# carry4985/ORB_SLAM2_MAP

Hardware: AMD Instinct MI355X
Metric: frames/sec ORB extract+match (640x480, 1000 feat) (higher is better)
Workload: dtype u8; 1 GPU; C2: synthetic 640x480 RGB-D stream, 1000 features, 8 levels, extract + BF-Hamming match of consecutive frames; resident_frame_pool=1024, sequences=1, parallelism=1 sequence per GPU, schedule_name=best, extraction_parts=1

## Files before the change

### include/orbgpu.h

```cpp
#ifndef ORBGPU_H
#define ORBGPU_H

#include <stddef.h>
#include <stdint.h>

#ifdef __cplusplus
extern "C" {
#endif

#define ORBGPU_ABI_VERSION 1
#define ORBGPU_MAX_LEVELS 16

typedef enum {
    ORBGPU_OK = 0,
    ORBGPU_EINVAL = -1,
    ORBGPU_ENOMEM = -2,
    ORBGPU_EHIP = -3,
    ORBGPU_ECAPACITY = -4,
    ORBGPU_ELEVEL = -5
} orbgpu_status;

const char *orbgpu_last_error_string(void);
int orbgpu_abi_version(void);
int orbgpu_device_count(void);
// ... 43 lines not shown
                         size_t stride, size_t frame_stride, orbgpu_keypoint *kps, uint8_t *desc, int32_t cap,
                         int32_t *n_out);

int orbgpu_extract_batch_device(orbgpu_extractor *h, const uint8_t *d_gray, int32_t batch, int32_t width,
                                int32_t height, size_t stride, size_t frame_stride, orbgpu_keypoint *d_kps,
                                uint8_t *d_desc, int32_t cap, int32_t *d_n_out, void *hip_stream);

int orbgpu_extractor_get_pyramid_level(orbgpu_extractor *h, int32_t frame, int32_t level, uint8_t *dst,
                                       size_t dst_stride, int32_t *width, int32_t *height);

enum {
    ORBGPU_DBG_PYRAMID_PADDED = 0,
    ORBGPU_DBG_BLURRED_PADDED = 1,
    ORBGPU_DBG_CANDIDATES = 2,
    ORBGPU_DBG_SELECTED = 3,
    ORBGPU_DBG_GRAPH_COUNTS = 4
};
int orbgpu_extractor_debug_read(orbgpu_extractor *h, int32_t what, int32_t frame, int32_t level, void *dst,
                                size_t dst_bytes, size_t *n, int32_t *aux);

int orbgpu_extractor_graph_state(const orbgpu_extractor *h, int32_t *state);
int orbgpu_extractor_debug_quadtree_config(const orbgpu_extractor *h, int32_t batch, int32_t *lds_keys, int32_t *threads,
                                           int32_t *lds_bytes);
int orbgpu_extractor_set_profiling(orbgpu_extractor *h, int32_t enable);
int orbgpu_extractor_set_concurrent_blur(orbgpu_extractor *h, int32_t enable);
int orbgpu_extractor_set_fast_early_out(orbgpu_extractor *h, int32_t enable);

int orbgpu_extractor_set_stage_signal(orbgpu_extractor *h, int32_t stage, void *hip_event);
int orbgpu_extractor_stage_count(void);
const char *orbgpu_extractor_stage_name(int32_t i);
int orbgpu_extractor_stage_times(orbgpu_extractor *h, float *ms_out);
// ... 388 lines not shown
```

### orb_slam2_map_amd/csrc/extractor.hip

```cpp
#include "common.h"

#include <atomic>
#include <chrono>
#include <thread>
#include <tuple>
#include <type_traits>
#include <utility>
#include "trig_base.h"
#include "pyramid_view.h"

#include <algorithm>
#include <cfloat>
#include <cmath>
#include <cstdlib>
#include <cstring>
#include <vector>

namespace orbgpu {

constexpr int EDGE = 19;
constexpr int BORDER0 = EDGE - 3;
constexpr int HALF_PATCH = 15;
constexpr int PATCH = 31;
constexpr float CELL_W = 30.f;
// ... 865 lines not shown
    __syncthreads();
    }
    __syncthreads();
    for (int i = tid; i < 4 * n_ini; i += 256)
        if (s_cnt[i])
            atomicAdd(&laux[1 + i], s_cnt[i]);
}

template <bool LDS_KEYS>
__global__ __launch_bounds__(QT_THREADS) void k_quadtree(const LevelGeom *__restrict__ geom,
                                                  const CellDesc *__restrict__ cells, int ncells_total,
                                                  const uint32_t *__restrict__ slots, size_t frame_slots,
                                                  int *__restrict__ cell_cnt,
                                                  uint32_t *__restrict__ dense_key,
                                                  uint16_t *__restrict__ dense_node,
                                                  uint32_t *__restrict__ sel, int sel_cap_total,
                                                  int *__restrict__ nsel, int *__restrict__ ncand, int nlevels,
                                                  int ncap, int t_ini, int kcap_arg, long long *dbg_t,
                                                  int *__restrict__ pre_aux )
{
#ifdef ORBGPU_QT_TIMING
    int dbg_k = 0;
#define QT_MARK(id) if (dbg_t && threadIdx.x == 0 && blockIdx.y == 0 && blockIdx.x == 0 && dbg_k < 500) { dbg_t[2 * dbg_k] = (id); dbg_t[2 * dbg_k + 1] = (long long)wall_clock64(); dbg_k++; }
#else
#define QT_MARK(id)
#endif

    extern __shared__ __align__(16) uint8_t smem[];
    __shared__ int s_tmp[16];
    const int kcap = LDS_KEYS ? kcap_arg : 0;
    __shared__ int s_n, s_phase, s_done, s_nexp, s_cut, s_nst, s_nk;
// ... 426 lines not shown
                nd[u] = node_of(i, key[u]);
            }
#pragma unroll
            for (int u = 0; u < QT_ILP; u++)
                if (i0 + u * nt < nkeys)
                    atomicMax(&best[nd[u]], best_of(key[u]));
        }
    }
    __syncthreads();
    uint32_t *osel = sel + (size_t)f * sel_cap_total + g.sel_off;
    const bool ok = done_cur != 2 && n <= g.sel_cap;
    for (int p = tid; p < n && ok; p += nt) {
        const unsigned long long b = best[p];
        const uint32_t yx = (uint32_t)((0xFFFFFFFFFFull - (b & 0xFFFFFFFFFFull)) & 0xFFFFFFull);
        osel[p] = (yx << 8) | (uint32_t)((b >> 40) - 1ull);
    }
    QT_MARK(4)
    if (tid == 0)
        nsel[(size_t)f * nlevels + level] = ok ? n : -1;
}

struct KpAux {
    int x, y, level;
    float angle;
    float ca, sb;
    int plane_off, pitch;
};

__device__ __forceinline__ float fast_atan2_deg(float y, float x)
{
// ... 15 lines not shown
        a = 180.f - a;
    if (y < 0)
        a = 360.f - a;
    return a;
}

struct UMax {
    int v[16];
};

constexpr int OR_ITERS = 4;
constexpr int OR_BATCH_MIN = 32;

__global__ __launch_bounds__(256) void k_orient(const uint8_t *__restrict__ pyr, size_t frame_pyr,
                                                const LevelGeom *__restrict__ geom, int nlevels,
                                                const uint32_t *__restrict__ sel, int sel_cap_total,
                                                const int *__restrict__ nsel, const uint32_t *__restrict__ orw,
                                                orbgpu_keypoint *__restrict__ kps, KpAux *__restrict__ aux,
                                                int cap, int *__restrict__ n_out, int iters, Src0 s0)
{
    __shared__ uint32_t W10[4 * 16 * 9], M01[4 * 16 * 9];
    __shared__ __align__(16) uint8_t stage[8][31 * 48];
    for (int i = threadIdx.x; i < 4 * 16 * 9; i += 256) {
        W10[i] = orw[i];
        M01[i] = orw[4 * 16 * 9 + i];
    }
    __syncthreads();

    const int hl = threadIdx.x & 31;
    int bx, f;
    xcd_frame_block(bx, f);
    f = serpentine(f);
    const int *ns = nsel + (size_t)f * nlevels;
    for (int it = 0; it < iters; it++) {
    const int slot = (bx * iters + it) * 8 + (threadIdx.x >> 5);
    int level = -1, j = 0, out_off = 0, total = 0, cnt_l = 0;
    bool bad = false;
// ... 11 lines not shown
            j = slot - so;
            out_off = total;
            cnt_l = c;
            g.plane_off = geom[l].plane_off;
            g.pitch = geom[l].pitch;
            g.sel_off = so;
            g.patch = geom[l].patch;
            g.scale = geom[l].scale;
        }
        total += max(c, 0);
    }
    if (slot == 0 && hl == 0)
        n_out[f] = bad ? -1 - total : (total > cap ? -1 - total : total);
    if (level < 0 || bad || total > cap || j >= cnt_l)
        continue;
    const uint32_t key = sel[(size_t)f * sel_cap_total + g.sel_off + j];
    const int x = key_x(key) + BORDER0, y = key_y(key) + BORDER0;
    const bool dir0 = s0.direct != 0 && level == 0;
    const int porg = dir0 ? 0 : EDGE, ppitch = dir0 ? (int)s0.pitch : g.pitch;
    const int xl = x + porg - HALF_PATCH;
    const int a = xl & 3;
    const int v = hl - HALF_PATCH;
    int m10 = 0, m01 = 0;
    {
        const uint8_t *base = (dir0 ? s0.p + (size_t)f * s0.frame_stride : pyr + (size_t)f * frame_pyr + g.plane_off) + (xl - a);
        struct __attribute__((packed, aligned(4))) Piece {
            uint32_t d[4];
        };
        const int lim = a == 2 ? 3 : (a == 3 ? 6 : -1);
        const uint8_t *rowbase = base + rowoff(y + porg - HALF_PATCH, ppitch);
        uint4 *pl = reinterpret_cast<uint4 *>(stage[threadIdx.x >> 5]);
// ... 42 lines not shown
    }
    if (hl == 0) {
        const float angle = fast_atan2_deg((float)m01, (float)m10);
        orbgpu_keypoint kp;
        kp.x = (float)x;
        kp.y = (float)y;
        if (level != 0) {
            kp.x *= g.scale;
            kp.y *= g.scale;
        }
        kp.size = (float)g.patch;
        kp.angle = angle;
        kp.response = (float)key_resp(key);
        kp.octave = level;
        kp.class_id = -1;
        kps[(size_t)f * cap + out_off + j] = kp;
        KpAux ax;
        ax.x = x + (dir0 ? BLUR0_OX - EDGE : 0);
        ax.y = y;
        ax.level = level;
        ax.plane_off = g.plane_off;
        ax.pitch = g.pitch;
        ax.angle = angle;
        aux[(size_t)f * cap + out_off + j] = ax;
    }
    }
}
__global__ __launch_bounds__(256) void k_trig(KpAux *__restrict__ aux, const int *__restrict__ n_out, int cap, TrigTable tt)
{
    const int f = blockIdx.y;
    const int i = blockIdx.x * 256 + threadIdx.x;
    if (i >= n_out[f])
        return;
    KpAux *a = aux + (size_t)f * cap + i;
    const float factorPI = (float)(3.14159265358979323846 / 180.f);
    const float angle = a->angle * factorPI;
    float c, s;
    orbgpu_trig_device(angle, tt, &c, &s);
    a->ca = c;
    a->sb = s;
}

constexpr int BLUR_ROWS = 30;

__device__ __forceinline__ void blur_hsum(uint32_t d0, uint32_t d1, uint32_t d2, uint32_t h[4])
{
#define W4(a, b, c, d) ((uint32_t)(a) | ((uint32_t)(b) << 8) | ((uint32_t)(c) << 16) | ((uint32_t)(d) << 24))
    h[0] = __builtin_amdgcn_udot4(d1, W4(55, 49, 34, 18), __builtin_amdgcn_udot4(d0, W4(0, 18, 34, 49), 0u, false), false);
    h[1] = __builtin_amdgcn_udot4(d2, W4(18, 0, 0, 0), __builtin_amdgcn_udot4(d1, W4(49, 55, 49, 34), __builtin_amdgcn_udot4(d0, W4(0, 0, 18, 34), 0u, false), false), false);
    h[2] = __builtin_amdgcn_udot4(d2, W4(34, 18, 0, 0), __builtin_amdgcn_udot4(d1, W4(34, 49, 55, 49), __builtin_amdgcn_udot4(d0, W4(0, 0, 0, 18), 0u, false), false), false);
    h[3] = __builtin_amdgcn_udot4(d2, W4(49, 34, 18, 0), __builtin_amdgcn_udot4(d1, W4(18, 34, 49, 55), 0u, false), false);
#undef W4
}

__device__ __forceinline__ uint32_t blur_vsum(const uint32_t A[4], const uint32_t C[4], const uint32_t E[4],
// ... 172 lines not shown
        B8_STEP(p5, p1, p3, p4, k + 5)
    }
#undef B8_PAIR
#undef B8_STEP
#undef B8_LOAD
#undef B8_HSUM
}

constexpr int DP_R = 18;
constexpr int DP_ROWS = 2 * DP_R + 1;
constexpr int DP_DW = 12;
constexpr int DP_BYTES = DP_ROWS * DP_DW * 4;

__global__ __launch_bounds__(256) void k_describe(const uint8_t *__restrict__ blur, size_t frame_pyr,
                                                  const LevelGeom *__restrict__ geom,
                                                  const KpAux *__restrict__ aux, const int *__restrict__ n_out,
                                                  int cap, const int8_t *__restrict__ pattern,
                                                  uint8_t *__restrict__ desc)
{
    __shared__ __align__(16) uint8_t patch[8][DP_BYTES];
    int bx, f;
    xcd_frame_block(bx, f);
    const int n = n_out[f];
    const int slot = threadIdx.x >> 5;
    const int kpi = bx * 8 + slot;
    if (kpi >= n)
        return;
    const int byte = threadIdx.x & 31;
    const KpAux a = aux[(size_t)f * cap + kpi];
    const uint4 pq0 = reinterpret_cast<const uint4 *>(pattern)[byte * 2];
    const uint4 pq1 = reinterpret_cast<const uint4 *>(pattern)[byte * 2 + 1];
    const uint32_t pw[8] = {pq0.x, pq0.y, pq0.z, pq0.w, pq1.x, pq1.y, pq1.z, pq1.w};
    const float ca = a.ca, sb = a.sb;
    const int xl = a.x + EDGE - DP_R;
    const int al = xl & 3;
    const uint8_t *fb = blur + (size_t)f * frame_pyr;
    const uint32_t vbase = (uint32_t)a.plane_off + (uint32_t)(a.y + EDGE - DP_R) * (uint32_t)a.pitch + (uint32_t)(xl - al);
    struct __attribute__((packed, aligned(4))) Piece {
        uint32_t d[4];
    };
    constexpr int NPIECE = DP_ROWS * 3, NK = (NPIECE + 31) / 32;
    Piece stage[NK];
#pragma unroll
    for (int k = 0; k < NK; k++) {
// ... 12 lines not shown
    constexpr float MAGIC = 12582912.0f;
    constexpr uint32_t BIAS = 0x400000u * (DP_DW * 4) + 0x4B400000u;
    const uint32_t kc = (uint32_t)(slot * DP_BYTES + DP_R * (DP_DW * 4) + DP_R + al) - BIAS;
    const uint8_t *lds = &patch[0][0];
    int val = 0;
#pragma unroll
    for (int k = 0; k < 8; k++) {
        const float x0 = (float)(int8_t)(pw[k] & 0xFF), y0 = (float)(int8_t)((pw[k] >> 8) & 0xFF);
        const float x1 = (float)(int8_t)((pw[k] >> 16) & 0xFF), y1 = (float)(int8_t)(pw[k] >> 24);
        const uint32_t r0b = __float_as_uint((x0 * sb + y0 * ca) + MAGIC), c0b = __float_as_uint((x0 * ca - y0 * sb) + MAGIC);
        const uint32_t r1b = __float_as_uint((x1 * sb + y1 * ca) + MAGIC), c1b = __float_as_uint((x1 * ca - y1 * sb) + MAGIC);
        const int t0 = lds[__umul24(r0b, DP_DW * 4) + c0b + kc];
        const int t1 = lds[__umul24(r1b, DP_DW * 4) + c1b + kc];
        val |= (t0 < t1) << k;
    }
    desc[((size_t)f * cap + kpi) * 32 + byte] = (uint8_t)val;
}

__global__ void k_unpack_keys(const uint32_t *__restrict__ keys, int n, int *__restrict__ out)
{
    int i = blockIdx.x * blockDim.x + threadIdx.x;
    if (i < n) {
        uint32_t k = keys[i];
        out[3 * i] = key_x(k);
        out[3 * i + 1] = key_y(k);
        out[3 * i + 2] = key_resp(k);
    }
}

static const int8_t k_pattern_host[1024] = {
#include "orbgpu_pattern.inc"
// ... 35 lines not shown
    int nlevels;
    float scale[ORBGPU_MAX_LEVELS], inv_scale[ORBGPU_MAX_LEVELS], sigma2[ORBGPU_MAX_LEVELS],
        inv_sigma2[ORBGPU_MAX_LEVELS];
    int quota[ORBGPU_MAX_LEVELS];
    UMax umax;
    int cfg_w = 0, cfg_h = 0, cfg_batch = 0;
    std::vector<LevelGeom> geom;
    std::vector<CellDesc> cells;
    StripGeom blur_geom;
    DetectGeom det_geom;
    size_t frame_pyr = 0, frame_slots = 0;
    int sel_cap_total = 0, ncap = 0, max_kp = 0;
    size_t qt_lds = 0;
    int qt_kcap = 0;
    DevBuf d_geom, d_cells, d_xtab, d_ytab, d_yrow, d_pattern, d_rstrip, d_rsel, d_rwt, d_ctab, d_bcol;
    DevBuf d_pyr, d_blur, d_slots, d_cellcnt, d_dkey, d_dnode, d_sel, d_nsel, d_ncand, d_aux;
    mutable DevBuf d_stereo;
    DevBuf d_qtaux;
    bool qt_prefilter = false;
    int max_slots_level = 0;
    DevBuf d_in, d_kps, d_desc, d_nout;
    void *h_pin = nullptr;
    size_t h_pin_bytes = 0;
    bool pinned_staging = true;
    DevBuf d_dbg;
    hipStream_t stream = nullptr;
    int last_batch = 0, last_cap = 0;
    static constexpr int PROF_SLOTS = 256;
    bool profiling = false;
    std::vector<hipEvent_t> ev;
    int prof_calls = 0;
// ... 7 lines not shown
    hipEvent_t stage_signal[8] = {nullptr, nullptr, nullptr, nullptr, nullptr, nullptr, nullptr, nullptr};
    hipEvent_t pipe_signal[8] = {};
    bool counters_dirty = false;
    bool force_batch_quadtree = false;
    bool concurrent_blur = false;
    hipStream_t side = nullptr;
    hipEvent_t ev_fork = nullptr, ev_fork0 = nullptr, ev_join = nullptr;
    bool qt_no_prefilter = false;
    int qt_keys_hook = -1;
    int fast_queue_cap = FD_QCAP;
    bool fast_early_out = false;
    int graph_state = 0;
    bool direct0_ok = false;
    bool no_early_blur0 = false;
    int direct0_min_batch = 8;
    bool no_direct0 = false;
    int rs_off_direct = 0;
    DetectGeom det_geom_direct;
    Src0 last_src = {nullptr, 0, 0u, 0};
    bool level0_materialized = true;
    TrigTable trig = {nullptr, nullptr, nullptr, 0u};

};

namespace orbgpu {

int trig_table_for_device(int device_id, TrigTable *out);

static void build_tables(orbgpu_extractor *e)
{
// ... 424 lines not shown
    RSV(e->d_xtab, sizeof(XTab) * std::max<size_t>(xtab.size(), 1));
    RSV(e->d_ytab, sizeof(YTab) * std::max<size_t>(ytab.size(), 1));
    RSV(e->d_yrow, sizeof(YRow) * std::max<size_t>(yrow.size(), 1));
    RSV(e->d_rstrip, sizeof(ResizeStrip) * std::max<size_t>(rstrip.size(), 1));
    RSV(e->d_rsel, sizeof(uint4) * std::max<size_t>(rsel.size(), 1));
    RSV(e->d_rwt, sizeof(uint4) * std::max<size_t>(rwt.size(), 1));
    RSV(e->d_pattern, 1024 + 2 * 4 * 16 * 9 * sizeof(uint32_t));
    const size_t B = (size_t)batch;
    RSV(e->d_pyr, e->frame_pyr * B);
    RSV(e->d_blur, e->frame_pyr * B);
    RSV(e->d_slots, sizeof(uint32_t) * e->frame_slots * B);
    RSV(e->d_cellcnt, sizeof(int) * (cells.size() + ORBGPU_MAX_LEVELS) * B);
    RSV(e->d_dkey, sizeof(uint32_t) * e->frame_slots * B);
    RSV(e->d_dnode, sizeof(uint16_t) * e->frame_slots * B);
    RSV(e->d_sel, sizeof(uint32_t) * (size_t)sel_off * B);
    RSV(e->d_nsel, sizeof(int) * nl * B);
    RSV(e->d_ncand, sizeof(int) * nl * B);
    RSV(e->d_qtaux, sizeof(int) * QT_AUX_FRAME * QT_BATCH_MIN);
#undef RSV
    ORBGPU_HIP_TRY(hipMemcpyAsync(e->d_geom.p, geom.data(), sizeof(LevelGeom) * nl, hipMemcpyHostToDevice, e->stream));
    ORBGPU_HIP_TRY(hipMemcpyAsync(e->d_cells.p, cells.data(), sizeof(CellDesc) * cells.size(), hipMemcpyHostToDevice, e->stream));
    ORBGPU_HIP_TRY(hipMemcpyAsync(e->d_ctab.p, ctab.data(), sizeof(ColumnInfo) * ctab.size(), hipMemcpyHostToDevice, e->stream));
    if (!bcol.empty())
        ORBGPU_HIP_TRY(hipMemcpyAsync(e->d_bcol.p, bcol.data(), sizeof(BorderCol) * bcol.size(), hipMemcpyHostToDevice, e->stream));
    e->border_fast = !bcol.empty();
    if (!xtab.empty()) {
        ORBGPU_HIP_TRY(hipMemcpyAsync(e->d_xtab.p, xtab.data(), sizeof(XTab) * xtab.size(), hipMemcpyHostToDevice, e->stream));
        ORBGPU_HIP_TRY(hipMemcpyAsync(e->d_ytab.p, ytab.data(), sizeof(YTab) * ytab.size(), hipMemcpyHostToDevice, e->stream));
        ORBGPU_HIP_TRY(hipMemcpyAsync(e->d_yrow.p, yrow.data(), sizeof(YRow) * yrow.size(), hipMemcpyHostToDevice, e->stream));
        ORBGPU_HIP_TRY(hipMemcpyAsync(e->d_rstrip.p, rstrip.data(), sizeof(ResizeStrip) * rstrip.size(), hipMemcpyHostToDevice, e->stream));
// ... 128 lines not shown
    if (e->blur_geom.first[nl] > strip0)
        L.launch(k_blur, dim3((e->blur_geom.first[nl] - strip0 + 255) / 256, batch), dim3(256), 0, pyr, blur,
                           e->frame_pyr, dg, e->blur_geom, strip0);
}

static int launch_pipeline(orbgpu_extractor *e, const uint8_t *d_gray, int batch, int w, int h, size_t stride,
                           size_t frame_stride, orbgpu_keypoint *d_kps, uint8_t *d_desc, int cap, int *d_n_out,
                           Launcher &L)
{
    hipStream_t st = L.st;
    const int nl = e->nlevels;
    const LevelGeom *dg = e->d_geom.as<LevelGeom>();
    uint8_t *pyr = e->d_pyr.as<uint8_t>();
    uint8_t *blur = e->d_blur.as<uint8_t>();
    int rc = e->d_aux.reserve(sizeof(KpAux) * (size_t)cap * batch);
    if (rc != ORBGPU_OK)
        return rc;
    const bool rec = L.graph != nullptr;
    const bool prof = !rec && e->profiling && e->prof_calls < orbgpu_extractor::PROF_SLOTS;
    if (prof && e->ev.empty()) {
        e->ev.resize((size_t)orbgpu_extractor::PROF_SLOTS * 2 * ST_COUNT, nullptr);
        for (auto &x : e->ev)
            ORBGPU_HIP_TRY(hipEventCreate(&x));
    }
    hipEvent_t *evs = prof ? &e->ev[(size_t)e->prof_calls * 2 * ST_COUNT] : nullptr;
#define BEGIN(stage, s) if (prof && (stage) == 0) ORBGPU_HIP_TRY(hipEventRecord(evs[0], s))
#define END(stage, s)                                                          \
    {                                                                          \
        if (prof)                                                              \
            ORBGPU_HIP_TRY(hipEventRecord(evs[1 + (stage)], s));               \
// ... 69 lines not shown
    {
        const int t_ini = std::max(e->prm.ini_th_fast, 1), t_min = std::max(e->prm.min_th_fast, 1);
        const DetectGeom &dgeo = direct ? e->det_geom_direct : e->det_geom;
        const int nwaves = (dgeo.first[nl] + FD_OWN - 1) / FD_OWN;
        L.launch(e->fast_early_out ? k_fast_detect<true> : k_fast_detect<false>, dim3((nwaves + 3) / 4, batch), dim3(256), 0, pyr, e->frame_pyr, dg,
                           dgeo, e->d_ctab.as<ColumnInfo>(), e->d_cells.as<CellDesc>(), (int)e->cells.size(),
                           e->d_slots.as<uint32_t>(), e->frame_slots, e->d_cellcnt.as<int>(), std::min(t_ini, t_min),
                           t_ini, e->fast_queue_cap, s0);
    }
    END(ST_FAST, st);
    BEGIN(ST_QUADTREE, st);
    if (batch >= QT_BATCH_MIN || e->force_batch_quadtree)
        L.launch(k_quadtree<false>, dim3(batch, nl), dim3(QT_THREADS_BATCH), e->qt_lds, dg,
                           e->d_cells.as<CellDesc>(), (int)e->cells.size(), e->d_slots.as<uint32_t>(), e->frame_slots,
                           e->d_cellcnt.as<int>(), e->d_dkey.as<uint32_t>(), e->d_dnode.as<uint16_t>(),
                           e->d_sel.as<uint32_t>(), e->sel_cap_total, e->d_nsel.as<int>(), e->d_ncand.as<int>(), nl,
                           e->ncap, std::max(e->prm.ini_th_fast, 1), 0, qt_dbg(), (int *)nullptr);
    else {
        if (e->qt_prefilter)
            L.launch(k_qt_prefilter, dim3(std::min((e->max_slots_level + QT_PRE_KEYS - 1) / QT_PRE_KEYS, QT_PRE_GRID), nl, batch), dim3(256), 0, dg, (int)e->cells.size(), e->d_slots.as<uint32_t>(), e->frame_slots, e->d_cellcnt.as<int>(),
                               e->d_dkey.as<uint32_t>(), e->d_qtaux.as<int>(), std::max(e->prm.ini_th_fast, 1));
        L.launch(k_quadtree<true>, dim3(batch, nl), dim3(w * h >= QT_LARGE_PIXELS ? QT_THREADS : QT_THREADS_SMALL), e->qt_lds + (size_t)e->qt_kcap * 6, dg,
                           e->d_cells.as<CellDesc>(), (int)e->cells.size(), e->d_slots.as<uint32_t>(), e->frame_slots,
                           e->d_cellcnt.as<int>(), e->d_dkey.as<uint32_t>(), e->d_dnode.as<uint16_t>(),
                           e->d_sel.as<uint32_t>(), e->sel_cap_total, e->d_nsel.as<int>(), e->d_ncand.as<int>(), nl,
                           e->ncap, std::max(e->prm.ini_th_fast, 1), e->qt_kcap, qt_dbg(),
                           e->qt_prefilter ? e->d_qtaux.as<int>() : (int *)nullptr);
    }
    if (!rec)
        ORBGPU_HIP_TRY(hipGetLastError());
    e->counters_dirty = false;
    END(ST_QUADTREE, st);
    BEGIN(ST_ORIENT, st);
    const int or_iters = batch >= OR_BATCH_MIN ? OR_ITERS : 1;
    L.launch(k_orient, dim3((e->sel_cap_total + 8 * or_iters - 1) / (8 * or_iters), batch), dim3(256), 0, pyr, e->frame_pyr, dg, nl,
                       e->d_sel.as<uint32_t>(), e->sel_cap_total, e->d_nsel.as<int>(),
                       reinterpret_cast<const uint32_t *>(e->d_pattern.as<uint8_t>() + 1024), d_kps,
                       e->d_aux.as<KpAux>(), cap, d_n_out, or_iters, s0);
    L.launch(k_trig, dim3((std::min(cap, e->max_kp) + 255) / 256, batch), dim3(256), 0,
                       e->d_aux.as<KpAux>(), d_n_out, cap, e->trig);
    END(ST_ORIENT, st);
    BEGIN(ST_DESCRIBE, st);
    if (side_blur)
        ORBGPU_HIP_TRY(hipStreamWaitEvent(st, e->ev_join, 0));
    L.launch(k_describe, dim3((std::min(cap, e->max_kp) + 7) / 8, batch), dim3(256), 0, blur,
                       e->frame_pyr, dg, e->d_aux.as<KpAux>(), d_n_out, cap, e->d_pattern.as<int8_t>(), d_desc);
    END(ST_DESCRIBE, st);
#undef BEGIN
#undef END
    if (!rec)
        ORBGPU_HIP_TRY(hipGetLastError());
    else if (L.err != hipSuccess) {
        set_error("recording the extraction graph: %s", hipGetErrorString(L.err));
        return ORBGPU_EHIP;
    }
    if (prof)
        e->prof_calls++;
    e->last_batch = batch;
    e->last_cap = cap;
    (void)w;
    (void)h;
// ... 51 lines not shown
    if (rc != ORBGPU_OK)
        return rc;
    orbgpu_extractor *e = new (std::nothrow) orbgpu_extractor();
    if (!e) {
        set_error("out of host memory");
        return ORBGPU_ENOMEM;
    }
    e->prm = *p;
    if (e->prm.max_batch < 1)
        e->prm.max_batch = 1;
    e->force_batch_quadtree = getenv("ORBGPU_DEBUG_QT_BATCH") != nullptr;
    e->qt_no_prefilter = getenv("ORBGPU_DEBUG_QT_NOPRE") != nullptr;
    if (const char *q = getenv("ORBGPU_DEBUG_QT_KEYS"))
        e->qt_keys_hook = std::max(atoi(q), 0);
    e->no_direct0 = getenv("ORBGPU_DEBUG_NO_DIRECT0") != nullptr;
    e->no_early_blur0 = getenv("ORBGPU_DEBUG_NO_EARLY_BLUR0") != nullptr;
    if (const char *q = getenv("ORBGPU_DEBUG_DIRECT0_MIN"))
        e->direct0_min_batch = std::max(atoi(q), 1);
    if (const char *q = getenv("ORBGPU_FAST_EARLY_OUT"))
        e->fast_early_out = atoi(q) != 0;
    e->pinned_staging = getenv("ORBGPU_DEBUG_NO_PINNED") == nullptr;
    if (getenv("ORBGPU_DEBUG_NO_GRAPH"))
        e->graph_state = -1;
    if (const char *q = getenv("ORBGPU_DEBUG_FAST_QUEUE"))
        e->fast_queue_cap = std::min(std::max(atoi(q), 0), FD_QCAP);
    e->nlevels = p->nlevels;
    build_tables(e);
    hipError_t he = hipStreamCreateWithFlags(&e->stream, hipStreamNonBlocking);
    if (he != hipSuccess) {
        set_error("hipStreamCreate: %s", hipGetErrorString(he));
// ... 7 lines not shown
        return rc;
    }
    *out = e;
    return ORBGPU_OK;
}

int orbgpu_extractor_destroy(orbgpu_extractor *e)
{
    std::lock_guard<std::mutex> lifecycle(orbgpu::lifecycle_mutex());
    if (!e)
        return ORBGPU_OK;
    (void)hipSetDevice(e->prm.device_id);
    (void)hipDeviceSynchronize();
    DevBuf *bufs[] = {&e->d_geom, &e->d_cells, &e->d_xtab, &e->d_ytab, &e->d_yrow, &e->d_pattern, &e->d_rstrip, &e->d_rsel,
                      &e->d_rwt, &e->d_ctab, &e->d_bcol, &e->d_pyr,
                      &e->d_blur, &e->d_slots, &e->d_cellcnt, &e->d_dkey, &e->d_dnode, &e->d_sel, &e->d_nsel,
                      &e->d_ncand, &e->d_aux, &e->d_in, &e->d_kps, &e->d_desc, &e->d_nout, &e->d_dbg, &e->d_qtaux, &e->d_stereo};
    for (DevBuf *b : bufs)
        b->release();
    for (auto &x : e->ev)
        if (x)
            (void)hipEventDestroy(x);
    if (e->graph_exec)
        (void)hipGraphExecDestroy(e->graph_exec);
    if (e->graph)
        (void)hipGraphDestroy(e->graph);
    if (e->h_pin)
        (void)hipHostFree(e->h_pin);
    if (e->stream)
        (void)hipStreamDestroy(e->stream);
    if (e->side)
        (void)hipStreamDestroy(e->side);
// ... 87 lines not shown
    const size_t img = (size_t)w * h;
    if (img * batch > e->d_in.bytes)
        forget_last_call(e);
    if ((rc = e->d_in.reserve(img * batch)) != ORBGPU_OK)
        return rc;
    if ((rc = e->d_kps.reserve(sizeof(orbgpu_keypoint) * (size_t)cap * batch)) != ORBGPU_OK)
        return rc;
    if ((rc = e->d_desc.reserve((size_t)32 * cap * batch)) != ORBGPU_OK)
        return rc;
    if ((rc = e->d_nout.reserve(sizeof(int) * batch)) != ORBGPU_OK)
        return rc;
    if ((rc = configure(e, w, h, std::max(batch, e->prm.max_batch))) != ORBGPU_OK)
        return rc;
    if ((rc = e->d_aux.reserve(sizeof(KpAux) * (size_t)cap * batch)) != ORBGPU_OK)
        return rc;
    uint8_t *pin_in = nullptr;
    int *pin_n = nullptr;
    orbgpu_keypoint *pin_k = nullptr;
    uint8_t *pin_d = nullptr;
    const size_t pin_need = ((img * batch + 255) & ~(size_t)255) + ((sizeof(int) * batch + 255) & ~(size_t)255) +
                            (sizeof(orbgpu_keypoint) + 32) * (size_t)cap * batch;
    if (e->pinned_staging && pin_need <= ((size_t)64 << 20)) {
        const size_t o_n = (img * batch + 255) & ~(size_t)255, o_k = o_n + ((sizeof(int) * batch + 255) & ~(size_t)255);
        const size_t o_d = o_k + sizeof(orbgpu_keypoint) * (size_t)cap * batch, need = o_d + (size_t)32 * cap * batch;
        if (need > e->h_pin_bytes) {
            if (e->h_pin)
                (void)hipHostFree(e->h_pin);
            e->h_pin = nullptr;
            e->h_pin_bytes = 0;
            ORBGPU_HIP_TRY(hipHostMalloc(&e->h_pin, need, hipHostMallocDefault));
// ... 2 lines not shown
        pin_in = static_cast<uint8_t *>(e->h_pin);
        pin_n = reinterpret_cast<int *>(pin_in + o_n);
        pin_k = reinterpret_cast<orbgpu_keypoint *>(pin_in + o_k);
        pin_d = pin_in + o_d;
        for (int f = 0; f < batch; f++)
            for (int y = 0; y < h; y++)
                memcpy(pin_in + img * f + (size_t)y * w, gray + frame_stride * f + stride * (size_t)y, (size_t)w);
        ORBGPU_HIP_TRY(hipMemcpyAsync(e->d_in.p, pin_in, img * batch, hipMemcpyHostToDevice, e->stream));
    } else
    for (int f = 0; f < batch; f++)
        ORBGPU_HIP_TRY(hipMemcpy2DAsync(e->d_in.as<uint8_t>() + img * f, (size_t)w, gray + frame_stride * f, stride,
                                        (size_t)w, (size_t)h, hipMemcpyHostToDevice, e->stream));
    uint64_t key = 1469598103934665603ull;
    for (uint64_t v : {(uint64_t)w, (uint64_t)h, (uint64_t)batch, (uint64_t)cap, (uint64_t)(uintptr_t)e->d_in.p,
                       (uint64_t)(uintptr_t)e->d_kps.p, (uint64_t)(uintptr_t)e->d_desc.p, (uint64_t)(uintptr_t)e->d_nout.p,
                       (uint64_t)(uintptr_t)e->d_pyr.p, (uint64_t)(uintptr_t)e->d_aux.p, (uint64_t)(uintptr_t)e->d_sel.p})
        key = (key ^ v) * 1099511628211ull;
    bool launched = false;
    if (!e->profiling && e->graph_state >= 0) {
        if (e->graph_exec && e->graph_key == key && !e->counters_dirty) {
            if (hipGraphLaunch(e->graph_exec, e->stream) == hipSuccess) {
                launched = true;
                e->last_src = e->graph_src;
                e->last_batch = e->graph_batch;
                e->last_cap = e->graph_cap;
                e->level0_materialized = !e->graph_src.direct;
                e->graph_replays++;
            } else
                e->graph_state = -1;
        } else if (e->graph_key == key) {
            hipGraph_t g = nullptr;
// ... 175 lines not shown
                    const int ai = (a.y - 3) / g.hcell, bi = (b.y - 3) / g.hcell;
                    const int aj = (a.x - 3) / g.wcell, bj = (b.x - 3) / g.wcell;
                    if (ai != bi)
                        return ai < bi;
                    if (aj != bj)
                        return aj < bj;
                    return a.y != b.y ? a.y < b.y : a.x < b.x;
                });
            }
        }
        *n = (size_t)cnt;
        if (aux)
            *aux = 0;
        return ORBGPU_OK;
    }
    set_error("unknown debug selector %d", what);
    return ORBGPU_EINVAL;
}

int orbgpu_extractor_set_stage_signal(orbgpu_extractor *e, int32_t stage, void *hip_event)
{
    ORBGPU_REQUIRE(e && stage >= 0 && stage < ST_COUNT, "bad stage");
    e->stage_signal[stage] = (hipEvent_t)hip_event;
    return ORBGPU_OK;
}

struct orbgpu_pipeline {
    std::vector<orbgpu_extractor *> part;
    std::vector<hipStream_t> stream;
    std::vector<hipEvent_t> ev_stage, ev_done;
// ... 213 lines not shown
```

### orb_slam2_map_amd/lib.py

```python
import ctypes as C
import os
import sys

import numpy as np

HERE = os.path.dirname(os.path.abspath(__file__))
LIB_PATH = os.path.join(HERE, "liborbgpu.so")

OK, EINVAL, ENOMEM, EHIP, ECAPACITY, ELEVEL = 0, -1, -2, -3, -4, -5
MAX_LEVELS = 16
GRID_COLS, GRID_ROWS = 64, 48
TH_HIGH, TH_LOW, HISTO_LENGTH = 100, 50, 30

KEYPOINT_DTYPE = np.dtype(
    [("x", "<f4"), ("y", "<f4"), ("size", "<f4"), ("angle", "<f4"), ("response", "<f4"),
     ("octave", "<i4"), ("class_id", "<i4")])
POINT_DTYPE = np.dtype([("x", "<f4"), ("y", "<f4"), ("z", "<f4"), ("rgba", "<u4")])

DBG_PYRAMID_PADDED, DBG_BLURRED_PADDED, DBG_CANDIDATES, DBG_SELECTED, DBG_GRAPH_COUNTS = 0, 1, 2, 3, 4


class OrbGpuError(RuntimeError):
    def __init__(self, status, msg):
        super().__init__("orbgpu status %d: %s" % (status, msg))
        self.status = status


class ExtractorParams(C.Structure):
    _fields_ = [("nfeatures", C.c_int32), ("scale_factor", C.c_float), ("nlevels", C.c_int32),
                ("ini_th_fast", C.c_int32), ("min_th_fast", C.c_int32), ("device_id", C.c_int32),
                ("max_batch", C.c_int32)]


class FrameView(C.Structure):
# ... 337 lines not shown
                                                 d_kps_ptr, d_desc_ptr, cap, d_nout_ptr, stream))

    def pyramid_level(self, frame, level):
        raw, pitch = self.debug_read(DBG_PYRAMID_PADDED, frame, level)
        img = raw.reshape(-1, pitch)
        return img

    def debug_read(self, what, frame, level):
        cap = 64 << 20
        buf = np.zeros(cap, np.uint8)
        n = C.c_size_t()
        aux = C.c_int32()
        check(self.L.orbgpu_extractor_debug_read(self.h, what, frame, level, _p(buf), cap, C.byref(n), C.byref(aux)))
        if what in (DBG_PYRAMID_PADDED, DBG_BLURRED_PADDED):
            return buf[:n.value].copy(), aux.value
        return buf[:n.value * 12].view(np.int32).reshape(-1, 3).copy(), 0

    def graph_counts(self):
        c = np.zeros(2, np.int32)
        n = C.c_size_t()
        check(self.L.orbgpu_extractor_debug_read(self.h, DBG_GRAPH_COUNTS, 0, 0, _p(c), c.nbytes, C.byref(n), None))
        return int(c[0]), int(c[1])

    def graph_state(self):
        v = C.c_int32()
        self.L.orbgpu_extractor_graph_state.argtypes = [C.c_void_p, C.c_void_p]
        check(self.L.orbgpu_extractor_graph_state(self.h, C.byref(v)))
        return v.value

    def quadtree_config(self, batch=1):
        a, b, c = C.c_int32(), C.c_int32(), C.c_int32()
# ... 937 lines not shown
```

Before: 286,400 frames/s.

## Visit keypoints in spatial tile order and fuse trig into orient kernel

The quadtree kernel now computes a rank-sort of selected keypoints by a tiled spatial key (64-pixel column tiles, then row) and writes a visit-order permutation. Orient and describe then process keypoints in that order while still writing results to their original slots, so that neighbouring threads touch nearby pyramid pixels and cache locality improves. The separate k_trig launch is removed: sin and cos are computed at the end of k_orient from shared memory. In exchange the rank sort costs O(n^2) shared-memory compares per level, there is an extra indirection buffer, and writes to kps, aux and desc become scattered.

Result: slower. 281,000 frames/s (-1.9%).

```diff
diff --git a/include/orbgpu.h b/include/orbgpu.h
--- a/include/orbgpu.h
+++ b/include/orbgpu.h
@@ -81,7 +81,8 @@
     ORBGPU_DBG_BLURRED_PADDED = 1,
     ORBGPU_DBG_CANDIDATES = 2,
     ORBGPU_DBG_SELECTED = 3,
-    ORBGPU_DBG_GRAPH_COUNTS = 4
+    ORBGPU_DBG_GRAPH_COUNTS = 4,
+    ORBGPU_DBG_VISIT_ORDER = 5
 };
 int orbgpu_extractor_debug_read(orbgpu_extractor *h, int32_t what, int32_t frame, int32_t level, void *dst,
                                 size_t dst_bytes, size_t *n, int32_t *aux);
diff --git a/orb_slam2_map_amd/csrc/extractor.hip b/orb_slam2_map_amd/csrc/extractor.hip
--- a/orb_slam2_map_amd/csrc/extractor.hip
+++ b/orb_slam2_map_amd/csrc/extractor.hip
@@ -903,7 +903,8 @@
                                                   int *__restrict__ cell_cnt,
                                                   uint32_t *__restrict__ dense_key,
                                                   uint16_t *__restrict__ dense_node,
-                                                  uint32_t *__restrict__ sel, int sel_cap_total,
+                                                  uint32_t *__restrict__ sel, uint16_t *__restrict__ ord, int kp_order,
+                                                  int sel_cap_total,
                                                   int *__restrict__ nsel, int *__restrict__ ncand, int nlevels,
                                                   int ncap, int t_ini, int kcap_arg, long long *dbg_t,
                                                   int *__restrict__ pre_aux )
@@ -1360,6 +1361,22 @@
         const unsigned long long b = best[p];
         const uint32_t yx = (uint32_t)((0xFFFFFFFFFFull - (b & 0xFFFFFFFFFFull)) & 0xFFFFFFull);
         osel[p] = (yx << 8) | (uint32_t)((b >> 40) - 1ull);
+        const uint32_t kx = ((yx & 0xFFFu) + (uint32_t)(BORDER0 + EDGE - HALF_PATCH)), ky = yx >> 12;
+        S.sa[p] = (int)(((kx >> 6) << 18) | (ky << 6) | (kx & 63u));
+    }
+    if (ok && kp_order != 0)
+        __syncthreads();
+    uint16_t *oord = ord + (size_t)f * sel_cap_total + g.sel_off;
+    for (int p = tid; p < n && ok; p += nt) {
+        int rank = p;
+        if (kp_order != 0) {
+            const int ka = S.sa[p];
+            rank = 0;
+#pragma unroll 4
+            for (int q = 0; q < n; q++)
+                rank += S.sa[q] < ka;
+        }
+        oord[rank] = (uint16_t)p;
     }
     QT_MARK(4)
     if (tid == 0)
@@ -1405,13 +1422,19 @@
 
 __global__ __launch_bounds__(256) void k_orient(const uint8_t *__restrict__ pyr, size_t frame_pyr,
                                                 const LevelGeom *__restrict__ geom, int nlevels,
-                                                const uint32_t *__restrict__ sel, int sel_cap_total,
+                                                const uint32_t *__restrict__ sel, const uint16_t *__restrict__ ord,
+                                                int sel_cap_total,
                                                 const int *__restrict__ nsel, const uint32_t *__restrict__ orw,
                                                 orbgpu_keypoint *__restrict__ kps, KpAux *__restrict__ aux,
-                                                int cap, int *__restrict__ n_out, int iters, Src0 s0)
+                                                int *__restrict__ vis, int cap, int *__restrict__ n_out, int iters, Src0 s0,
+                                                TrigTable tt)
 {
     __shared__ uint32_t W10[4 * 16 * 9], M01[4 * 16 * 9];
     __shared__ __align__(16) uint8_t stage[8][31 * 48];
+    __shared__ __align__(16) KpAux s_aux[8 * OR_ITERS];
+    __shared__ int s_idx[8 * OR_ITERS];
+    if (threadIdx.x < 8 * OR_ITERS)
+        s_idx[threadIdx.x] = -1;
     for (int i = threadIdx.x; i < 4 * 16 * 9; i += 256) {
         W10[i] = orw[i];
         M01[i] = orw[4 * 16 * 9 + i];
@@ -1453,7 +1476,8 @@
         n_out[f] = bad ? -1 - total : (total > cap ? -1 - total : total);
     if (level < 0 || bad || total > cap || j >= cnt_l)
         continue;
-    const uint32_t key = sel[(size_t)f * sel_cap_total + g.sel_off + j];
+    const int jv = min((int)ord[(size_t)f * sel_cap_total + g.sel_off + j], cnt_l - 1);
+    const uint32_t key = sel[(size_t)f * sel_cap_total + g.sel_off + jv];
     const int x = key_x(key) + BORDER0, y = key_y(key) + BORDER0;
     const bool dir0 = s0.direct != 0 && level == 0;
     const int porg = dir0 ? 0 : EDGE, ppitch = dir0 ? (int)s0.pitch : g.pitch;
@@ -1526,7 +1550,8 @@
         kp.response = (float)key_resp(key);
         kp.octave = level;
         kp.class_id = -1;
-        kps[(size_t)f * cap + out_off + j] = kp;
+        kps[(size_t)f * cap + out_off + jv] = kp;
+        vis[(size_t)f * cap + out_off + j] = out_off + jv;
         KpAux ax;
         ax.x = x + (dir0 ? BLUR0_OX - EDGE : 0);
         ax.y = y;
@@ -1534,23 +1559,21 @@
         ax.plane_off = g.plane_off;
         ax.pitch = g.pitch;
         ax.angle = angle;
-        aux[(size_t)f * cap + out_off + j] = ax;
-    }
-    }
-}
-__global__ __launch_bounds__(256) void k_trig(KpAux *__restrict__ aux, const int *__restrict__ n_out, int cap, TrigTable tt)
-{
-    const int f = blockIdx.y;
-    const int i = blockIdx.x * 256 + threadIdx.x;
-    if (i >= n_out[f])
-        return;
-    KpAux *a = aux + (size_t)f * cap + i;
-    const float factorPI = (float)(3.14159265358979323846 / 180.f);
-    const float angle = a->angle * factorPI;
-    float c, s;
-    orbgpu_trig_device(angle, tt, &c, &s);
-    a->ca = c;
-    a->sb = s;
+        ax.ca = ax.sb = 0.f;
+        s_aux[it * 8 + (threadIdx.x >> 5)] = ax;
+        s_idx[it * 8 + (threadIdx.x >> 5)] = out_off + jv;
+    }
+    }
+    __syncthreads();
+    if (threadIdx.x < 8 * iters) {
+        const int idx = s_idx[threadIdx.x];
+        if (idx >= 0) {
+            KpAux ax = s_aux[threadIdx.x];
+            const float factorPI = (float)(3.14159265358979323846 / 180.f);
+            orbgpu_trig_device(ax.angle * factorPI, tt, &ax.ca, &ax.sb);
+            aux[(size_t)f * cap + idx] = ax;
+        }
+    }
 }
 
 constexpr int BLUR_ROWS = 30;
@@ -1753,7 +1776,8 @@
 
 __global__ __launch_bounds__(256) void k_describe(const uint8_t *__restrict__ blur, size_t frame_pyr,
                                                   const LevelGeom *__restrict__ geom,
-                                                  const KpAux *__restrict__ aux, const int *__restrict__ n_out,
+                                                  const KpAux *__restrict__ aux, const int *__restrict__ vis,
+                                                  const int *__restrict__ n_out,
                                                   int cap, const int8_t *__restrict__ pattern,
                                                   uint8_t *__restrict__ desc)
 {
@@ -1766,7 +1790,8 @@
     if (kpi >= n)
         return;
     const int byte = threadIdx.x & 31;
-    const KpAux a = aux[(size_t)f * cap + kpi];
+    const int idx = min(max(vis[(size_t)f * cap + kpi], 0), n - 1);
+    const KpAux a = aux[(size_t)f * cap + idx];
     const uint4 pq0 = reinterpret_cast<const uint4 *>(pattern)[byte * 2];
     const uint4 pq1 = reinterpret_cast<const uint4 *>(pattern)[byte * 2 + 1];
     const uint32_t pw[8] = {pq0.x, pq0.y, pq0.z, pq0.w, pq1.x, pq1.y, pq1.z, pq1.w};
@@ -1809,7 +1834,7 @@
         const int t1 = lds[__umul24(r1b, DP_DW * 4) + c1b + kc];
         val |= (t0 < t1) << k;
     }
-    desc[((size_t)f * cap + kpi) * 32 + byte] = (uint8_t)val;
+    desc[((size_t)f * cap + idx) * 32 + byte] = (uint8_t)val;
 }
 
 __global__ void k_unpack_keys(const uint32_t *__restrict__ keys, int n, int *__restrict__ out)
@@ -1875,7 +1900,7 @@
     size_t qt_lds = 0;
     int qt_kcap = 0;
     DevBuf d_geom, d_cells, d_xtab, d_ytab, d_yrow, d_pattern, d_rstrip, d_rsel, d_rwt, d_ctab, d_bcol;
-    DevBuf d_pyr, d_blur, d_slots, d_cellcnt, d_dkey, d_dnode, d_sel, d_nsel, d_ncand, d_aux;
+    DevBuf d_pyr, d_blur, d_slots, d_cellcnt, d_dkey, d_dnode, d_sel, d_ord, d_nsel, d_ncand, d_aux, d_vis;
     mutable DevBuf d_stereo;
     DevBuf d_qtaux;
     bool qt_prefilter = false;
@@ -1913,6 +1938,7 @@
     bool direct0_ok = false;
     bool no_early_blur0 = false;
     int direct0_min_batch = 8;
+    int kp_order = 1;
     bool no_direct0 = false;
     int rs_off_direct = 0;
     DetectGeom det_geom_direct;
@@ -2367,6 +2393,7 @@
     RSV(e->d_dkey, sizeof(uint32_t) * e->frame_slots * B);
     RSV(e->d_dnode, sizeof(uint16_t) * e->frame_slots * B);
     RSV(e->d_sel, sizeof(uint32_t) * (size_t)sel_off * B);
+    RSV(e->d_ord, sizeof(uint16_t) * (size_t)sel_off * B);
     RSV(e->d_nsel, sizeof(int) * nl * B);
     RSV(e->d_ncand, sizeof(int) * nl * B);
     RSV(e->d_qtaux, sizeof(int) * QT_AUX_FRAME * QT_BATCH_MIN);
@@ -2525,6 +2552,8 @@
     uint8_t *pyr = e->d_pyr.as<uint8_t>();
     uint8_t *blur = e->d_blur.as<uint8_t>();
     int rc = e->d_aux.reserve(sizeof(KpAux) * (size_t)cap * batch);
+    if (rc == ORBGPU_OK)
+        rc = e->d_vis.reserve(sizeof(int) * (size_t)cap * batch);
     if (rc != ORBGPU_OK)
         return rc;
     const bool rec = L.graph != nullptr;
@@ -2624,7 +2653,7 @@
         L.launch(k_quadtree<false>, dim3(batch, nl), dim3(QT_THREADS_BATCH), e->qt_lds, dg,
                            e->d_cells.as<CellDesc>(), (int)e->cells.size(), e->d_slots.as<uint32_t>(), e->frame_slots,
                            e->d_cellcnt.as<int>(), e->d_dkey.as<uint32_t>(), e->d_dnode.as<uint16_t>(),
-                           e->d_sel.as<uint32_t>(), e->sel_cap_total, e->d_nsel.as<int>(), e->d_ncand.as<int>(), nl,
+                           e->d_sel.as<uint32_t>(), e->d_ord.as<uint16_t>(), e->kp_order, e->sel_cap_total, e->d_nsel.as<int>(), e->d_ncand.as<int>(), nl,
                            e->ncap, std::max(e->prm.ini_th_fast, 1), 0, qt_dbg(), (int *)nullptr);
     else {
         if (e->qt_prefilter)
@@ -2633,7 +2662,7 @@
         L.launch(k_quadtree<true>, dim3(batch, nl), dim3(w * h >= QT_LARGE_PIXELS ? QT_THREADS : QT_THREADS_SMALL), e->qt_lds + (size_t)e->qt_kcap * 6, dg,
                            e->d_cells.as<CellDesc>(), (int)e->cells.size(), e->d_slots.as<uint32_t>(), e->frame_slots,
                            e->d_cellcnt.as<int>(), e->d_dkey.as<uint32_t>(), e->d_dnode.as<uint16_t>(),
-                           e->d_sel.as<uint32_t>(), e->sel_cap_total, e->d_nsel.as<int>(), e->d_ncand.as<int>(), nl,
+                           e->d_sel.as<uint32_t>(), e->d_ord.as<uint16_t>(), e->kp_order, e->sel_cap_total, e->d_nsel.as<int>(), e->d_ncand.as<int>(), nl,
                            e->ncap, std::max(e->prm.ini_th_fast, 1), e->qt_kcap, qt_dbg(),
                            e->qt_prefilter ? e->d_qtaux.as<int>() : (int *)nullptr);
     }
@@ -2644,17 +2673,15 @@
     BEGIN(ST_ORIENT, st);
     const int or_iters = batch >= OR_BATCH_MIN ? OR_ITERS : 1;
     L.launch(k_orient, dim3((e->sel_cap_total + 8 * or_iters - 1) / (8 * or_iters), batch), dim3(256), 0, pyr, e->frame_pyr, dg, nl,
-                       e->d_sel.as<uint32_t>(), e->sel_cap_total, e->d_nsel.as<int>(),
+                       e->d_sel.as<uint32_t>(), e->d_ord.as<uint16_t>(), e->sel_cap_total, e->d_nsel.as<int>(),
                        reinterpret_cast<const uint32_t *>(e->d_pattern.as<uint8_t>() + 1024), d_kps,
-                       e->d_aux.as<KpAux>(), cap, d_n_out, or_iters, s0);
-    L.launch(k_trig, dim3((std::min(cap, e->max_kp) + 255) / 256, batch), dim3(256), 0,
-                       e->d_aux.as<KpAux>(), d_n_out, cap, e->trig);
+                       e->d_aux.as<KpAux>(), e->d_vis.as<int>(), cap, d_n_out, or_iters, s0, e->trig);
     END(ST_ORIENT, st);
     BEGIN(ST_DESCRIBE, st);
     if (side_blur)
         ORBGPU_HIP_TRY(hipStreamWaitEvent(st, e->ev_join, 0));
     L.launch(k_describe, dim3((std::min(cap, e->max_kp) + 7) / 8, batch), dim3(256), 0, blur,
-                       e->frame_pyr, dg, e->d_aux.as<KpAux>(), d_n_out, cap, e->d_pattern.as<int8_t>(), d_desc);
+                       e->frame_pyr, dg, e->d_aux.as<KpAux>(), e->d_vis.as<int>(), d_n_out, cap, e->d_pattern.as<int8_t>(), d_desc);
     END(ST_DESCRIBE, st);
 #undef BEGIN
 #undef END
@@ -2736,6 +2763,7 @@
     if (const char *q = getenv("ORBGPU_DEBUG_QT_KEYS"))
         e->qt_keys_hook = std::max(atoi(q), 0);
     e->no_direct0 = getenv("ORBGPU_DEBUG_NO_DIRECT0") != nullptr;
+    e->kp_order = getenv("ORBGPU_DEBUG_NO_KP_ORDER") ? 0 : 1;
     e->no_early_blur0 = getenv("ORBGPU_DEBUG_NO_EARLY_BLUR0") != nullptr;
     if (const char *q = getenv("ORBGPU_DEBUG_DIRECT0_MIN"))
         e->direct0_min_batch = std::max(atoi(q), 1);
@@ -2773,8 +2801,8 @@
     (void)hipDeviceSynchronize();
     DevBuf *bufs[] = {&e->d_geom, &e->d_cells, &e->d_xtab, &e->d_ytab, &e->d_yrow, &e->d_pattern, &e->d_rstrip, &e->d_rsel,
                       &e->d_rwt, &e->d_ctab, &e->d_bcol, &e->d_pyr,
-                      &e->d_blur, &e->d_slots, &e->d_cellcnt, &e->d_dkey, &e->d_dnode, &e->d_sel, &e->d_nsel,
-                      &e->d_ncand, &e->d_aux, &e->d_in, &e->d_kps, &e->d_desc, &e->d_nout, &e->d_dbg, &e->d_qtaux, &e->d_stereo};
+                      &e->d_blur, &e->d_slots, &e->d_cellcnt, &e->d_dkey, &e->d_dnode, &e->d_sel, &e->d_ord, &e->d_nsel,
+                      &e->d_ncand, &e->d_aux, &e->d_vis, &e->d_in, &e->d_kps, &e->d_desc, &e->d_nout, &e->d_dbg, &e->d_qtaux, &e->d_stereo};
     for (DevBuf *b : bufs)
         b->release();
     for (auto &x : e->ev)
@@ -2892,6 +2920,8 @@
         return rc;
     if ((rc = e->d_aux.reserve(sizeof(KpAux) * (size_t)cap * batch)) != ORBGPU_OK)
         return rc;
+    if ((rc = e->d_vis.reserve(sizeof(int) * (size_t)cap * batch)) != ORBGPU_OK)
+        return rc;
     uint8_t *pin_in = nullptr;
     int *pin_n = nullptr;
     orbgpu_keypoint *pin_k = nullptr;
@@ -2924,7 +2954,8 @@
     uint64_t key = 1469598103934665603ull;
     for (uint64_t v : {(uint64_t)w, (uint64_t)h, (uint64_t)batch, (uint64_t)cap, (uint64_t)(uintptr_t)e->d_in.p,
                        (uint64_t)(uintptr_t)e->d_kps.p, (uint64_t)(uintptr_t)e->d_desc.p, (uint64_t)(uintptr_t)e->d_nout.p,
-                       (uint64_t)(uintptr_t)e->d_pyr.p, (uint64_t)(uintptr_t)e->d_aux.p, (uint64_t)(uintptr_t)e->d_sel.p})
+                       (uint64_t)(uintptr_t)e->d_pyr.p, (uint64_t)(uintptr_t)e->d_aux.p, (uint64_t)(uintptr_t)e->d_sel.p,
+                       (uint64_t)(uintptr_t)e->d_ord.p, (uint64_t)(uintptr_t)e->d_vis.p})
         key = (key ^ v) * 1099511628211ull;
     bool launched = false;
     if (!e->profiling && e->graph_state >= 0) {
@@ -3130,6 +3161,22 @@
             *aux = 0;
         return ORBGPU_OK;
     }
+    if (what == ORBGPU_DBG_VISIT_ORDER) {
+        int cnt = 0, per_level[ORBGPU_MAX_LEVELS];
+        ORBGPU_HIP_TRY(hipMemcpy(per_level, e->d_nsel.as<int>() + (size_t)frame * e->nlevels, sizeof(int) * e->nlevels, hipMemcpyDeviceToHost));
+        for (int l = 0; l < e->nlevels; l++) {
+            ORBGPU_REQUIRE(per_level[l] >= 0, "stage reported failure (%d)", per_level[l]);
+            cnt += per_level[l];
+        }
+        ORBGPU_REQUIRE(cnt <= e->last_cap, "the last call's capacity (%d) was below the frame's %d key points", e->last_cap, cnt);
+        ORBGPU_REQUIRE(dst_bytes >= (size_t)cnt * 4, "dst too small (%zu needed)", (size_t)cnt * 4);
+        if (cnt > 0)
+            ORBGPU_HIP_TRY(hipMemcpy(dst, e->d_vis.as<int>() + (size_t)e->last_cap * frame, (size_t)cnt * 4, hipMemcpyDeviceToHost));
+        *n = (size_t)cnt;
+        if (aux)
+            *aux = 0;
+        return ORBGPU_OK;
+    }
     set_error("unknown debug selector %d", what);
     return ORBGPU_EINVAL;
 }
diff --git a/orb_slam2_map_amd/lib.py b/orb_slam2_map_amd/lib.py
--- a/orb_slam2_map_amd/lib.py
+++ b/orb_slam2_map_amd/lib.py
@@ -17,7 +17,7 @@
      ("octave", "<i4"), ("class_id", "<i4")])
 POINT_DTYPE = np.dtype([("x", "<f4"), ("y", "<f4"), ("z", "<f4"), ("rgba", "<u4")])
 
-DBG_PYRAMID_PADDED, DBG_BLURRED_PADDED, DBG_CANDIDATES, DBG_SELECTED, DBG_GRAPH_COUNTS = 0, 1, 2, 3, 4
+DBG_PYRAMID_PADDED, DBG_BLURRED_PADDED, DBG_CANDIDATES, DBG_SELECTED, DBG_GRAPH_COUNTS, DBG_VISIT_ORDER = 0, 1, 2, 3, 4, 5
 
 
 class OrbGpuError(RuntimeError):
@@ -385,7 +385,12 @@
         check(self.L.orbgpu_extractor_debug_read(self.h, what, frame, level, _p(buf), cap, C.byref(n), C.byref(aux)))
         if what in (DBG_PYRAMID_PADDED, DBG_BLURRED_PADDED):
             return buf[:n.value].copy(), aux.value
+        if what == DBG_VISIT_ORDER:
+            return buf[:n.value * 4].view(np.int32).copy(), 0
         return buf[:n.value * 12].view(np.int32).reshape(-1, 3).copy(), 0
+
+    def visit_order(self, frame):
+        return self.debug_read(DBG_VISIT_ORDER, frame, 0)[0]
 
     def graph_counts(self):
         c = np.zeros(2, np.int32)
```
